# ohsnyt/bzip2-rust

Hardware: NVIDIA B200
Metric: compress_MBps_level9_byte_identical (higher is better)
Workload: dtype u8

## Files before the change

bzip2_rust_b200/csrc/bwt.cu:

```cuda
#include "common.cuh"
#include "sweep.cuh"

namespace {

constexpr int FB = 20;
constexpr u64 FMASK = (1ull << FB) - 1;
static_assert(BZ2B200_MAX_BLOCK < (1u << FB) - 1, "packed list fields are 20 bits");

constexpr int RT_IPT = 8;
constexpr int RT = BZ_THREADS * RT_IPT;
__device__ __forceinline__ u32 padi(u32 i) { return i + (i >> 5); }
constexpr int RT_PAD = RT + RT / 32 + 1;

#ifndef BZ_LW
#define BZ_LW 3072
#endif
constexpr int LW = BZ_LW;
constexpr int LIPT = LW / BZ_THREADS;
#ifndef BZ_LCAP
#define BZ_LCAP 1024
#endif
constexpr int LCAP = BZ_LCAP;
constexpr int LTILE = LW - LCAP;
#ifndef BZ_SCAP
// ... 60 lines not shown
            v.b = BSUM ? v.b + ob : max(v.b, ob);
            v.c += __shfl_xor_sync(0xffffffffu, v.c, o);
        }
        ex.a = max(ex.a, v.a); ex.b = BSUM ? ex.b + v.b : max(ex.b, v.b); ex.c += v.c;
        if (incm) break;
        hi -= 32;
    }
    Tri inc; inc.a = max(ex.a, agg.a); inc.b = BSUM ? ex.b + agg.b : max(ex.b, agg.b); inc.c = ex.c + agg.c;
    if (lane == 0) st_vol64(st + t, tri_pack(2, inc));
    return ex;
}

struct RefineArgs {
    const u8 *T; const u32 *len;
    const u32 *cnt;
    u32 *SA; u32 *RANK;
    const u64 *LIN; u64 *LOUT;
    u32 *cnt_out;
    u64 *LOUT2;
    u32 *cnt_out2;
    u64 *tstate;
    u32 *ticket;
    u32 stride, rtiles, tiles_x, nblk, group;
    u32 depth_after;
};

__device__ __forceinline__ bool ticket_tile(const RefineArgs &a, u32 *s_ticket, u32 &b, u32 &t) {
    if (threadIdx.x == 0) *s_ticket = atomicAdd(a.ticket, 1u);
    __syncthreads();
    u32 ticket = *s_ticket;
    u32 per_group = a.group * a.tiles_x;
    u32 g = ticket / per_group, r = ticket - g * per_group;
    t = r / a.group;
    b = g * a.group + (r - t * a.group);
    return b < a.nblk;
}

#ifndef BZ_REFINE_MINB
#define BZ_REFINE_MINB 5
#endif
__global__ void __launch_bounds__(BZ_THREADS, BZ_REFINE_MINB) k_init_ranks(RefineArgs a) {
    __shared__ u64 sk[RT + 2];
    __shared__ __align__(8) u8 fl[RT + 8];
    __shared__ u32 hd[RT_PAD];
    __shared__ u16 ls[RT];
    __shared__ int wsi[8];
    __shared__ u32 wsu[8];
    __shared__ u32 s_ticket;
    __shared__ Tri s_ex;
    __shared__ int s_big[2];
    u32 b, t;
    if (!ticket_tile(a, &s_ticket, b, t)) return;
    const u32 n = a.len[b];
    const u32 base = t * RT;
    if (base >= n) return;
    const int tid = threadIdx.x;
    const size_t ob = (size_t)b * a.stride;
    const u8 *Tb = a.T + ob;
    const u32 *sa = a.SA + ob;
    u32 s[RT_IPT];
#pragma unroll
    for (int r = 0; r < RT_IPT; r++) {
        u32 e = r * BZ_THREADS + tid, j = base + e;
        s[r] = 0;
        if (j < n) { s[r] = __ldg(sa + j); sk[e + 1] = rot_key8(Tb, n, s[r]); }
    }
    if (tid == 0 && base > 0) sk[0] = rot_key8(Tb, n, sa[base - 1]);
    if (tid == 32 && base + RT < n) sk[RT + 1] = rot_key8(Tb, n, sa[base + RT]);
    __syncthreads();
    for (u32 e = tid; e <= RT; e += BZ_THREADS) {
        u32 j = base + e;
        fl[e] = (j == 0 || j >= n || sk[e + 1] != sk[e]) ? 1 : 0;
    }
    __syncthreads();
    const u32 eb = tid * RT_IPT;
    const u64 f8 = *(const u64 *)(fl + eb);
    const u32 f9 = fl[eb + 8];
    u32 fm = 0;
#pragma unroll
    for (int r = 0; r < RT_IPT; r++) fm |= (u32)((f8 >> (8 * r)) & 1) << r;
    int last = -1;
    u32 hmask = 0, umask = 0;
#pragma unroll
    for (int r = 0; r < RT_IPT; r++) {
        u32 j = base + eb + r;
        bool h = (fm >> r) & 1;
        bool hn = (r == RT_IPT - 1) ? (f9 != 0) : ((fm >> (r + 1)) & 1);
        if (j < n) {
            if (h) { last = (int)j; hmask |= 1u << r; }
            if (!(h && hn)) umask |= 1u << r;
        }
    }
    int tl, fe;
    int head = block_excl_max(last, wsi, tl);
    int nxa = block_excl_min_rev(fm ? (int)(eb + __ffs(fm) - 1) : 0x7fffffff, wsi, fe);
    const bool cont = fl[RT] == 0;
    if (tid == 64) {
        int big = 0;
        if (fl[0] == 0) {
            if (fe == 0x7fffffff && cont) big = 1;
            else {
                long long E = (long long)base + (fe == 0x7fffffff ? (int)RT : fe);
                long long q = E - 1 - LCAP;
                if (q >= (long long)base) big = 1;
                else if (q >= 0) big = rot_key8(Tb, n, sa[q]) == sk[1];
            }
        }
        s_big[0] = big;
    }
    if (tid == 96) {
        int big = 0;
        if (cont) {
            if (tl < 0) big = 1;
            else {
                u32 P = (u32)tl + LCAP;
                if (P < base + RT) big = 1;
                else if (P < n) big = rot_key8(Tb, n, sa[P]) == sk[RT];
            }
        }
        s_big[1] = big;
    }
    __syncthreads();
    const int nx_out = f9 ? (int)(eb + 8) : (nxa != 0x7fffffff ? nxa : (cont ? 0x7fffffff : (int)RT));
    u32 bmask = 0, nloc = 0, nbig = 0;
#pragma unroll
    for (int r = 0; r < RT_IPT; r++) {
        if ((umask >> r) & 1) {
            u32 below = fm & ((2u << r) - 1u);
            int hh = below ? (int)(base + eb + 31 - __clz(below)) : head;
            u32 above = fm >> (r + 1);
            int nx = above ? (int)(eb + r + __ffs(above)) : nx_out;
            bool big;
            if (hh < 0) big = s_big[0] != 0;
            else if (nx == 0x7fffffff) big = s_big[1] != 0;
            else big = (int)base + nx - hh > LCAP;
            if (big) { bmask |= 1u << r; nbig++; } else nloc++;
        }
    }
    u32 tot;
    u32 kk = block_excl_sum(nloc | (nbig << 16), wsu, tot);
    const u32 tloc = tot & 0xffffu, tbig = tot >> 16;
    if (tid < 32) {
        Tri agg; agg.a = tl; agg.b = (int)tbig; agg.c = tloc;
        Tri ex = tile_lookback<true>(a.tstate + (size_t)b * a.rtiles, t, agg);
        if (tid == 0) {
            s_ex = ex;
            if (base + RT >= n) {
                bool done = a.depth_after >= n;
                a.cnt_out[b] = done ? 0u : ex.c + tloc;
                a.cnt_out2[b] = done ? 0u : (u32)ex.b + tbig;
            }
        }
    }
    __syncthreads();
    head = max(head, s_ex.a);
    u32 kl = kk & 0xffffu, kb = kk >> 16;
#pragma unroll
    for (int r = 0; r < RT_IPT; r++) {
        u32 e = eb + r;
        if ((hmask >> r) & 1) head = (int)(base + e);
        hd[padi(e)] = (u32)head;
        u16 v = 0xffff;
        if ((umask >> r) & 1) v = ((bmask >> r) & 1) ? (u16)(0x8000u | kb++) : (u16)(kl++);
        ls[e] = v;
    }
    __syncthreads();
    u32 *rank = a.RANK + ob;
    u64 *lout = a.LOUT + ob + s_ex.c;
    u64 *lout2 = a.LOUT2 + ob + (u32)s_ex.b;
#pragma unroll
    for (int r = 0; r < RT_IPT; r++) {
        u32 e = r * BZ_THREADS + tid, j = base + e;
        if (j < n) {
            u32 h = hd[padi(e)];
            rank[s[r]] = h;
            u32 slot = ls[e];
            if (slot != 0xffffu) {
                u64 v = ((u64)h << (2 * FB)) | s[r];
                if (slot & 0x8000u) lout2[slot & 0x7fffu] = v; else lout[slot] = v;
            }
        }
    }
}

template <bool HIST>
__global__ void __launch_bounds__(BZ_THREADS) k_list_key(const u32 *cntp, const u32 *len, const u32 *RANK, u64 *LIST,
                                                         u32 *counts, u32 stride, u32 h) {
    u32 b = blockIdx.y, cnt = cntp[b], n = len[b];
    u32 base = blockIdx.x * BZ_TILE;
    if (base >= cnt) return;
    __shared__ u32 hist[HIST ? 5 : 1][256];
    if (HIST) {
        for (int i = threadIdx.x; i < 5 * 256; i += BZ_THREADS) (&hist[0][0])[i] = 0;
        __syncthreads();
    }
    size_t ob = (size_t)b * stride;
    u64 *list = LIST + ob;
    const u32 *rank = RANK + ob;
    u32 hh = h >= n ? h % n : h;
#pragma unroll 4
    for (int r = 0; r < BZ_IPT; r++) {
        u32 k = base + r * BZ_THREADS + threadIdx.x;
        if (k < cnt) {
            u64 x = list[k];
            u32 p = (u32)(x & FMASK) + hh;
            if (p >= n) p -= n;
            x = (x & ~(FMASK << FB)) | ((u64)__ldg(rank + p) << FB);
            list[k] = x;
            if (HIST) {
#pragma unroll
                for (int q = 0; q < 5; q++) atomicAdd(&hist[q][(u32)(x >> (FB + 8 * q)) & 255u], 1u);
            }
        }
// ... 50 lines not shown
    u32 f9 = fl[eb + 8];
    int la = -1, lb = -1; u32 unres = 0;
    u32 smask = 0, gmask = 0, umask = 0;
#pragma unroll
    for (int r = 0; r < RT_IPT; r++) {
        u32 k = base + eb + r;
        u32 f = (u32)(f8 >> (8 * r)) & 3u;
        u32 fn = (r == RT_IPT - 1) ? f9 : ((u32)(f8 >> (8 * r + 8)) & 3u);
        if (k < cnt) {
            if (f & 2) { la = (int)k; gmask |= 1u << r; }
            if (f & 1) { lb = (int)k; smask |= 1u << r; }
            if (!((f & 1) && (fn & 1))) { unres++; umask |= 1u << r; }
        }
    }
    int ta, tb; u32 tu;
    int kg = block_excl_max(la, wsi, ta);
    int ks = block_excl_max(lb, wsi, tb);
    u32 ko = block_excl_sum(unres, wsu, tu);
    if (tid < 32) {
        Tri agg; agg.a = ta; agg.b = tb; agg.c = tu;
        Tri ex = tile_lookback(a.tstate + (size_t)b * a.rtiles, t, agg);
        if (tid == 0) {
            s_ex = ex;
            if (base + RT >= cnt) a.cnt_out[b] = (a.depth_after >= a.len[b]) ? 0u : ex.c + tu;
        }
    }
    __syncthreads();
    kg = max(kg, s_ex.a); ks = max(ks, s_ex.b);
    const u32 kbase = s_ex.c;
#pragma unroll
    for (int r = 0; r < RT_IPT; r++) {
        u32 e = eb + r;
        if ((gmask >> r) & 1) kg = (int)(base + e);
        if ((smask >> r) & 1) ks = (int)(base + e);
        kgs[padi(e)] = (u32)kg; kss[padi(e)] = (u32)ks;
        ls[e] = ((umask >> r) & 1) ? (u16)(ko++) : (u16)0xffff;
    }
    __syncthreads();
    u32 *sa = a.SA + ob, *rank = a.RANK + ob;
    u64 *lout = a.LOUT + ob + kbase;
#pragma unroll
    for (int r = 0; r < RT_IPT; r++) {
        u32 e = r * BZ_THREADS + tid, k = base + e;
        if (k < cnt) {
            u32 g = (u32)(x[r] >> (2 * FB));
            u32 s = (u32)(x[r] & FMASK);
            u32 kgv = kgs[padi(e)], ksv = kss[padi(e)];
            u32 nh = g + (ksv - kgv);
            sa[g + (k - kgv)] = s;
            rank[s] = nh;
            u32 slot = ls[e];
            if (slot != 0xffffu) lout[slot] = ((u64)nh << (2 * FB)) | s;
        }
    }
}

constexpr size_t LOC_K_BYTES = (size_t)LW * 4;
constexpr size_t LOC_I_BYTES = ((size_t)LWH * 2 + 15) & ~(size_t)15;
constexpr size_t LOC_G_BYTES = ((size_t)LWP * 4 + 15) & ~(size_t)15;
constexpr size_t LOC_U_BYTES = ((size_t)LWH * 2 + 15) & ~(size_t)15;
constexpr size_t LOC_W_BYTES = (size_t)(LW * 4 > 8 * 256 * 4 ? LW * 4 : 8 * 256 * 4);
constexpr size_t LOC_SMEM = LOC_K_BYTES + 2 * LOC_I_BYTES + LOC_G_BYTES + LOC_U_BYTES + LOC_W_BYTES;
static_assert(LOC_K_BYTES + 2 * LOC_I_BYTES >= (size_t)LW * 8, "staging area");
#ifndef BZ_LOCAL_MINB
#define BZ_LOCAL_MINB 3
#endif
__global__ void __launch_bounds__(BZ_THREADS, BZ_LOCAL_MINB) k_refine_local(RefineArgs a, u32 *err) {
    extern __shared__ __align__(16) u8 loc_smem[];
    u32 *K = (u32 *)loc_smem;
    u16 *IDXA = (u16 *)(loc_smem + LOC_K_BYTES);
    u16 *IDXB = (u16 *)(loc_smem + LOC_K_BYTES + LOC_I_BYTES);
    u32 *GSE = (u32 *)(loc_smem + LOC_K_BYTES + 2 * LOC_I_BYTES);
    u16 *UP = (u16 *)((u8 *)GSE + LOC_G_BYTES);
    u32 *wh = (u32 *)((u8 *)UP + LOC_U_BYTES);
    __shared__ u16 MG_GS[LW / (SCAP + 1) + 4], MG_MB[LW / (SCAP + 1) + 4];
    __shared__ int wsi[8];
    __shared__ u32 wsu[8];
    __shared__ u32 s_ticket, s_prevhead;
    __shared__ Tri s_ex;
    u32 b, t;
    if (!ticket_tile(a, &s_ticket, b, t)) return;
    const u32 cnt = a.cnt[b];
    const u32 base = t * LTILE;
    const int tid = threadIdx.x, lane = tid & 31, w = tid >> 5;
    if (cnt == 0 && t == 0 && tid == 0) a.cnt_out[b] = 0;
    if (base >= cnt) return;
    const size_t ob = (size_t)b * a.stride;
    const u64 *lin = a.LIN + ob + base;
// ... 167 lines not shown
            pk = k2;
            occ |= 1u << r;
        }
        occ &= (1u << LIPT) - 1u;
        const u32 own = sfm & ((1u << LIPT) - 1u);
        const u32 tm = occ & ~(own & (sfm >> 1));
        const int pin = block_excl_max(own ? (int)(eb + 31 - __clz(own)) : -1, wsi, dummy);
        u32 run = block_excl_sum((u32)__popc(tm), wsu, tu);
        int ps = pin;
#pragma unroll 4
        for (int r = 0; r < LIPT; r++) {
            u32 p = eb + r;
            if ((own >> r) & 1u) ps = (int)p;
            wh[p] = run | ((p - (u32)ps) << 12) | (((tm >> r) & 1u) << 31);
            run += (tm >> r) & 1u;
        }
    }
    __syncthreads();
    if (tid < 32) {
        Tri agg; agg.a = -1; agg.b = -1; agg.c = tu;
        Tri ex = tile_lookback(a.tstate + (size_t)b * a.rtiles, t, agg);
        if (tid == 0) {
            s_ex = ex;
            if (base + LTILE >= cnt) a.cnt_out[b] = (a.depth_after >= a.len[b]) ? 0u : ex.c + tu;
        }
    }
    u64 *stg = (u64 *)loc_smem;
    u32 *sa = a.SA + ob, *rank = a.RANK + ob;
#pragma unroll 2
    for (int r = 0; r < LIPT; r++) {
        u32 p = r * BZ_THREADS + tid;
        u32 e = UP[padh(p)];
        if (e != 0xffffu) {
            u32 gs = GSE[padi(e)] & 0xffffu;
            u32 v = wh[p];
            u64 x = __ldg(lin + e);
            u32 head = (u32)(x >> (2 * FB)), s = (u32)(x & FMASK);
            u32 off = p - gs;
            u32 nh = head + off - ((v >> 12) & 0x7ffffu);
            sa[head + off] = s;
            rank[s] = nh;
            if (v >> 31) stg[v & 0xfffu] = ((u64)nh << (2 * FB)) | s;
        }
    }
    __syncthreads();
    u64 *lout = a.LOUT + ob + s_ex.c;
    for (u32 q = tid; q < tu; q += BZ_THREADS) lout[q] = stg[q];
// ... 64 lines not shown
        if (e_ != cudaSuccess) { ctx->fail("kernel launch", e_, __FILE__, __LINE__); return BZ2B200_E_CUDA; } \
    } while (0)

int bz_bwt_batch(bz2b200_ctx *ctx, const Batch &B, u8 *d_bwt, u32 *d_key, u32 *d_usedbits) {
    if (B.nblk == 0) return BZ2B200_OK;
    if (B.max_n > BZ2B200_MAX_BLOCK || ((uintptr_t)B.T & 7u) || (B.stride & 7u)) { ctx->err = "bwt: bad batch geometry"; return BZ2B200_E_ARG; }
    cudaStream_t st = ctx->stream;
    const u64 ne_act = B.total_n;
    const size_t ne = (size_t)B.nblk * B.stride;
    const u32 min_tile = BZ_THREADS * 8;
    const u32 tiles_min = B.stride / min_tile;
    const u32 DSTRIDE = 8 * 256;
    const u32 NTICKET = 512;
    BZ_CHECK(ctx->d_SA.ensure(ne * 4));
    BZ_CHECK(ctx->d_SA2.ensure(ne * 4));
    BZ_CHECK(ctx->d_RANK.ensure(ne * 4));
    BZ_CHECK(ctx->d_KEYA.ensure(ne * 8));
    BZ_CHECK(ctx->d_KEYB.ensure(ne * 8));
    BZ_CHECK(ctx->d_thist.ensure((size_t)B.nblk * tiles_min * 256 * 4));
    BZ_CHECK(ctx->d_tagg.ensure((size_t)B.nblk * tiles_min * 8));
    BZ_CHECK(ctx->d_VALA.ensure(ne * 8));
    BZ_CHECK(ctx->d_VALB.ensure(ne * 8));
    BZ_CHECK(ctx->d_cnt.ensure((size_t)B.nblk * 4 * 4 + 16));
    BZ_CHECK(ctx->d_R.ensure(((size_t)B.nblk * DSTRIDE + NTICKET) * 4));
    BZ_CHECK(ctx->h_small.ensure((size_t)B.nblk * 8 + 64));
    u32 *d_sais = ctx->d_cnt.as<u32>() + (size_t)B.nblk * 4;
    BZ_CHECK(cudaMemsetAsync(d_sais, 0, 8, ctx->stream));
    if (!ctx->loc_attr_done) {
        BZ_CHECK(cudaFuncSetAttribute(k_refine_local, cudaFuncAttributeMaxDynamicSharedMemorySize, (int)LOC_SMEM));
        ctx->loc_attr_done = true;
    }
    u32 *SAa = ctx->d_SA.as<u32>(), *SAb = ctx->d_SA2.as<u32>(), *RANK = ctx->d_RANK.as<u32>();
    u64 *L0 = ctx->d_KEYA.as<u64>(), *L1 = ctx->d_KEYB.as<u64>();
    u64 *G0 = ctx->d_VALA.as<u64>(), *G1 = ctx->d_VALB.as<u64>();
    u32 *tstate = ctx->d_thist.as<u32>();
    u64 *rstate = ctx->d_tagg.as<u64>();
    u32 *dcounts = ctx->d_R.as<u32>();
    u32 *tickets = dcounts + (size_t)B.nblk * DSTRIDE;
    const size_t rstate_bytes = (size_t)B.nblk * tiles_min * 8;

    BZ_CHECK(cudaMemsetAsync(dcounts, 0, ((size_t)B.nblk * DSTRIDE + NTICKET) * 4, st));
    BZ_CHECK(cudaMemsetAsync(tstate, 0, (size_t)B.nblk * tiles_min * 256 * 4, st));
    u32 epoch = 0, tk = 0;
    dim3 gfull((B.max_n + BZ_TILE - 1) / BZ_TILE, B.nblk);
    static const u32 group_knob = [] { const char *e = getenv("BZ2B200_REFINE_GROUP"); u32 g = e ? (u32)atoi(e) : 4u; return g < 1 ? 1u : g; }();
    const u32 group = group_knob < (u32)B.nblk ? group_knob : (u32)B.nblk;

    ctx->prof_begin(K_BYTE_HIST, ne_act); sweep::k_byte_hist<<<gfull, BZ_THREADS, 0, st>>>(B.T, B.len, dcounts, B.stride, DSTRIDE); LAUNCH_OK();
    ctx->prof_begin(K_REF_PATH, (u64)B.nblk * 5000); k_ref_path<<<B.nblk, 128, 0, st>>>(B.T, B.len, B.stride, d_sais); LAUNCH_OK();
    if (d_usedbits) { ctx->prof_begin(K_USED, (u64)B.nblk * 1024); k_used_from_hist<<<B.nblk, 256, 0, st>>>(dcounts, DSTRIDE, d_usedbits); LAUNCH_OK(); }
    ctx->prof_begin(K_DIGIT_SCAN, (u64)B.nblk * DSTRIDE * 4); sweep::k_digit_scan<<<B.nblk * 8, 256, 0, st>>>(dcounts); LAUNCH_OK();
    u32 *bufs[2] = {SAa, SAb};
    const u32 *src = nullptr;
    for (int p = 0; p < 8; p++) {
        sweep::Args a{};
        a.T = B.T; a.len = B.len; a.cnt = B.len; a.in = src; a.out = bufs[p & 1];
        a.stride = B.stride; a.off = 7 - p; a.nblk = (u32)B.nblk;
        epoch++;
        a.dbase = dcounts; a.dbase_stride = DSTRIDE; a.tstate = tstate; a.ticket = tickets + tk++; a.epoch = epoch;
        if ((p & 1) == 0) { ctx->prof_begin(K_SWEEP_GATHER, ne_act * 9); sweep::launch<sweep::M_GATHER>(a, B.max_n, st); }
        else { ctx->prof_begin(K_SWEEP_CARRY, ne_act * 8); sweep::launch<sweep::M_CARRY>(a, B.max_n, st); }
        LAUNCH_OK();
        src = bufs[p & 1];
    }
    u32 *SA = bufs[1];

    u32 *cntL_cur = ctx->d_cnt.as<u32>(), *cntL_nxt = cntL_cur + B.nblk;
    u32 *cntB_cur = cntL_nxt + B.nblk, *cntB_nxt = cntB_cur + B.nblk;
    RefineArgs ra{};
    ra.T = B.T; ra.len = B.len; ra.SA = SA; ra.RANK = RANK; ra.stride = B.stride; ra.rtiles = tiles_min;
    ra.nblk = (u32)B.nblk; ra.group = group; ra.tstate = rstate;
    {
        BZ_CHECK(cudaMemsetAsync(rstate, 0, rstate_bytes, st));
        ra.cnt = B.len; ra.LIN = nullptr; ra.LOUT = L0; ra.cnt_out = cntL_cur; ra.LOUT2 = G0; ra.cnt_out2 = cntB_cur;
        ra.ticket = tickets + tk++;
        ra.tiles_x = (B.max_n + RT - 1) / RT; ra.depth_after = 8;
        u32 grid = ((ra.nblk + group - 1) / group) * group * ra.tiles_x;
        ctx->prof_begin(K_INIT_RANKS, ne_act * 16); k_init_ranks<<<grid, BZ_THREADS, 0, st>>>(ra); LAUNCH_OK();
    }

    u32 *h_cnt = ctx->h_small.as<u32>();
    const int passes = 5;
    u64 rounds = 0, listsum = 0, bigsum = 0;
    for (u32 h = 8;; h *= 2) {
        BZ_CHECK(cudaMemcpyAsync(h_cnt + 2 * B.nblk, d_sais, 8, cudaMemcpyDeviceToHost, st));
        BZ_CHECK(cudaMemcpyAsync(h_cnt, cntL_cur, (size_t)B.nblk * 4, cudaMemcpyDeviceToHost, st));
        BZ_CHECK(cudaMemcpyAsync(h_cnt + B.nblk, cntB_cur, (size_t)B.nblk * 4, cudaMemcpyDeviceToHost, st));
        BZ_CHECK(cudaStreamSynchronize(st));
        u32 maxl = 0, maxb = 0;
        u64 lsum = 0, bsum = 0;
        for (int b = 0; b < B.nblk; b++) {
            if (h_cnt[b] > maxl) maxl = h_cnt[b];
            if (h_cnt[B.nblk + b] > maxb) maxb = h_cnt[B.nblk + b];
            lsum += h_cnt[b]; bsum += h_cnt[B.nblk + b];
        }
        listsum += lsum + bsum; bigsum += bsum;
        if (maxl == 0 && maxb == 0) break;
        if (h >= (1u << 30)) { ctx->err = "bwt: doubling did not terminate"; return BZ2B200_E_CUDA; }
        rounds++;
        if (tk + (u32)passes + 3 > NTICKET) { BZ_CHECK(cudaMemsetAsync(tickets, 0, NTICKET * 4, st)); tk = 0; }
        if (maxl) {
            dim3 gl((maxl + BZ_TILE - 1) / BZ_TILE, B.nblk);
            ctx->prof_begin(K_LIST_KEY, lsum * 20); k_list_key<false><<<gl, BZ_THREADS, 0, st>>>(cntL_cur, B.len, RANK, L0, nullptr, B.stride, h); LAUNCH_OK();
            BZ_CHECK(cudaMemsetAsync(rstate, 0, rstate_bytes, st));
            ra.cnt = cntL_cur; ra.LIN = L0; ra.LOUT = L1; ra.cnt_out = cntL_nxt; ra.LOUT2 = nullptr; ra.cnt_out2 = nullptr;
            ra.ticket = tickets + tk++;
            ra.tiles_x = (maxl + LTILE - 1) / LTILE; ra.depth_after = 2 * h;
            u32 grid = ((ra.nblk + group - 1) / group) * group * ra.tiles_x;
            ctx->prof_begin(K_REFINE_LOCAL, lsum * 24); k_refine_local<<<grid, BZ_THREADS, LOC_SMEM, st>>>(ra, d_sais + 1); LAUNCH_OK();
            { u64 *tl = L0; L0 = L1; L1 = tl; }
        } else BZ_CHECK(cudaMemsetAsync(cntL_nxt, 0, (size_t)B.nblk * 4, st));
        if (maxb) {
            dim3 gl((maxb + BZ_TILE - 1) / BZ_TILE, B.nblk);
            BZ_CHECK(cudaMemsetAsync(dcounts, 0, (size_t)B.nblk * DSTRIDE * 4, st));
            ctx->prof_begin(K_LIST_KEY, bsum * 20); k_list_key<true><<<gl, BZ_THREADS, 0, st>>>(cntB_cur, B.len, RANK, G0, dcounts, B.stride, h); LAUNCH_OK();
            ctx->prof_begin(K_DIGIT_SCAN, (u64)B.nblk * DSTRIDE * 4); sweep::k_digit_scan<<<B.nblk * 8, 256, 0, st>>>(dcounts); LAUNCH_OK();
            if (epoch + (u32)passes > 254) {
                BZ_CHECK(cudaMemsetAsync(tstate, 0, (size_t)B.nblk * tiles_min * 256 * 4, st));
                epoch = 0;
            }
            for (int p = 0; p < passes; p++) {
                sweep::Args a{};
                a.T = B.T; a.len = B.len; a.cnt = cntB_cur; a.in = G0; a.out = G1;
                a.stride = B.stride; a.shift = FB + 8 * p; a.nblk = (u32)B.nblk;
                epoch++;
                a.dbase = dcounts + p * 256; a.dbase_stride = DSTRIDE; a.tstate = tstate; a.ticket = tickets + tk++; a.epoch = epoch;
                ctx->prof_begin(K_SWEEP_LIST, bsum * 16); sweep::launch<sweep::M_LIST>(a, maxb, st); LAUNCH_OK();
                u64 *tl = G0; G0 = G1; G1 = tl;
            }
            BZ_CHECK(cudaMemsetAsync(rstate, 0, rstate_bytes, st));
            ra.cnt = cntB_cur; ra.LIN = G0; ra.LOUT = G1; ra.cnt_out = cntB_nxt; ra.LOUT2 = nullptr; ra.cnt_out2 = nullptr;
            ra.ticket = tickets + tk++;
            ra.tiles_x = (maxb + RT - 1) / RT; ra.depth_after = 2 * h;
            u32 grid = ((ra.nblk + group - 1) / group) * group * ra.tiles_x;
            ctx->prof_begin(K_LIST_REFINE, bsum * 24); k_list_refine<<<grid, BZ_THREADS, 0, st>>>(ra); LAUNCH_OK();
            { u64 *tl = G0; G0 = G1; G1 = tl; }
        } else BZ_CHECK(cudaMemsetAsync(cntB_nxt, 0, (size_t)B.nblk * 4, st));
        { u32 *tc = cntL_cur; cntL_cur = cntL_nxt; cntL_nxt = tc; }
        { u32 *tc = cntB_cur; cntB_cur = cntB_nxt; cntB_nxt = tc; }
    }
    if (h_cnt[2 * B.nblk + 1]) { ctx->err = "bwt: a local group exceeded its capacity"; return BZ2B200_E_CUDA; }
    ctx->prof_begin(K_BWT_OUT, ne_act * 6); k_bwt_out<<<gfull, BZ_THREADS, 0, st>>>(B.T, B.len, SA, RANK, d_bwt, d_key, B.stride); LAUNCH_OK();
    ctx->bwt_stats[0] = (u64)B.nblk; ctx->bwt_stats[1] = ne_act; ctx->bwt_stats[2] = rounds; ctx->bwt_stats[3] = listsum;
    ctx->bwt_stats[4] = h_cnt[2 * B.nblk];
    ctx->bwt_stats[5] += h_cnt[2 * B.nblk];
    ctx->bwt_stats[6] += (u64)B.nblk;
    ctx->bwt_stats[7] = bigsum;
    return BZ2B200_OK;
}
```

bzip2_rust_b200/csrc/common.cuh:

```cuda
#pragma once
#include <cuda_runtime.h>
#include <stdint.h>
#include <stddef.h>
#include <mutex>
#include <string>
#include <vector>
#include <new>
#include "../../include/bz2b200.h"

typedef uint8_t u8;
typedef uint16_t u16;
typedef uint32_t u32;
typedef uint64_t u64;

#define BZ_CHECK(call)                                                                     \
    do {                                                                                   \
        cudaError_t e_ = (call);                                                           \
        if (e_ != cudaSuccess) {                                                           \
            ctx->fail(#call, e_, __FILE__, __LINE__);                                      \
            return BZ2B200_E_CUDA;                                                         \
        }                                                                                  \
    } while (0)

#define BZ_API_TRY try {
// ... 27 lines not shown
        return e;
    }
    void release() { if (p) cudaFreeHost(p); p = nullptr; cap = 0; }
    template <class T> T *as() const { return (T *)p; }
};

constexpr int BZ_THREADS = 256;
constexpr int BZ_IPT = 16;
constexpr int BZ_TILE = BZ_THREADS * BZ_IPT;
constexpr int BZ_GROUP = 50;
constexpr int BZ_MAXSYM = 258;

struct Batch {
    int nblk;
    u32 stride;
    u32 tiles;
    u32 max_n;
    int nbits;
    const u8 *T;
    const u32 *len;
    u64 total_n;
};

enum KernelId { K_RADIX_HIST0, K_RADIX_SCAN, K_RADIX_SCATTER0, K_REF_PATH, K_BYTE_HIST, K_DIGIT_SCAN, K_SWEEP_GATHER, K_SWEEP_CARRY, K_SWEEP_LIST, K_INIT_RANKS, K_LIST_KEY, K_LIST_REFINE, K_REFINE_LOCAL, K_BWT_OUT, K_USED, K_MTF_SUMMARY, K_MTF_SCAN, K_MTF_EMIT, K_HUF_INIT, K_HUF_SELECT, K_HUF_LENGTHS, K_HUF_GBITS, K_HUF_LAYOUT, K_HUF_EMIT, K_RLE_SCAN, K_RLE_CHAIN, K_RLE_EMIT, K_CRC_PIECES, K_CRC_FINAL, K_CONCAT, K_FOOTER, K_DEC_MISC, K_DEC_MAGIC, K_DEC_HEADER, K_DEC_JUMPS, K_DEC_BOUNDS, K_DEC_SYMS, K_DEC_CHUNKS, K_DEC_EXPAND, K_DEC_CHUNK_SCAN, K_IBWT_CHASE, K_IBWT_RANK, K_IBWT_WRITE, K_DEC_RLE1_COUNT, K_DEC_RLE1_WRITE, K_COUNT };
static const char *const kKernelNames[] = { "k_radix_hist0", "k_radix_scan", "k_radix_scatter0", "k_ref_path", "k_byte_hist", "k_digit_scan", "k_sweep_gather", "k_sweep_carry", "k_sweep_list", "k_init_ranks", "k_list_key", "k_list_refine", "k_refine_local", "k_bwt_out", "k_used", "k_mtf_summary", "k_mtf_scan", "k_mtf_emit", "k_huf_init", "k_huf_select", "k_huf_lengths", "k_huf_gbits", "k_huf_layout", "k_huf_emit", "k_rle_scan", "k_rle_chain", "k_rle_emit", "k_crc_pieces", "k_crc_final", "k_concat", "k_footer", "k_dec_misc", "k_dec_find_magic", "k_dec_header", "k_dec_jumps", "k_dec_bounds", "k_dec_syms", "k_dec_chunks", "k_dec_expand", "k_dec_chunk_scan", "k_ibwt_chase", "k_ibwt_rank", "k_ibwt_write", "k_dec_rle1_count", "k_dec_rle1_write" };

struct KStat { double ms = 0; u64 launches = 0; u64 bytes = 0; };
struct PendingEv { int id; u64 bytes; cudaEvent_t a, b; };

struct Arrival {
    std::vector<cudaEvent_t> *ev;
    size_t chunk;
    size_t win_off;
    size_t waited;
};

struct ShardPlan {
    bool scanned = false;
    const u8 *d_win = nullptr; size_t win_lo = 0, win_len = 0, n_total = 0; int level = 0;
    bool planned = false;
    bool eof = false; u32 off_from = 0, stop_rel = 0, s0 = 0, nb = 0;
};

struct bz2b200_ctx {
    int device = 0;
    ShardPlan shard;
    cudaStream_t stream = nullptr;
    cudaStream_t s_up = nullptr, s_down = nullptr;
// ... 157 lines not shown
```

bzip2_rust_b200/csrc/sweep.cuh:

```cuda
#pragma once
#include "common.cuh"
#include <stdlib.h>
#include <type_traits>

namespace sweep {

enum { M_GATHER = 0, M_LIST = 1, M_CARRY = 2 };

struct Args {
    const u8 *T; const u32 *len;
    const u32 *cnt;
    const void *in; void *out;
    const u32 *dbase;
    u32 dbase_stride;
    u32 *tstate;
    u32 *ticket;
    u32 stride;
    u32 rtiles;
    u32 epoch;
    u32 tiles_x;
    u32 nblk;
    u32 group;
    int off;
    int shift;
};

__device__ __forceinline__ u32 ld_vol(const u32 *p) {
    u32 v;
    asm volatile("ld.volatile.global.u32 %0, [%1];" : "=r"(v) : "l"(p));
    return v;
}
__device__ __forceinline__ void st_vol(u32 *p, u32 v) { asm volatile("st.volatile.global.u32 [%0], %1;" ::"l"(p), "r"(v) : "memory"); }

#ifndef BZ_SWEEP_TMA
#define BZ_SWEEP_TMA 0
#endif
__device__ __forceinline__ u32 smem_u32(const void *p) { return (u32)__cvta_generic_to_shared(p); }
__device__ __forceinline__ void mbar_init(u64 *bar, u32 count) {
    asm volatile("mbarrier.init.shared::cta.b64 [%0], %1;" ::"r"(smem_u32(bar)), "r"(count) : "memory");
    asm volatile("fence.mbarrier_init.release.cluster;" ::: "memory");
}
__device__ __forceinline__ void bulk_load(void *dst, const void *src, u32 bytes, u64 *bar) {
    asm volatile("mbarrier.arrive.expect_tx.shared::cta.b64 _, [%0], %1;" ::"r"(smem_u32(bar)), "r"(bytes) : "memory");
    asm volatile("cp.async.bulk.shared::cluster.global.mbarrier::complete_tx::bytes [%0], [%1], %2, [%3];"
// ... 152 lines not shown
__global__ void __launch_bounds__(BZ_THREADS, min_ctas(MODE, IPT)) k_sweep(Args a) {
    typedef typename Types<MODE>::Stage S;
    constexpr int TILE = BZ_THREADS * IPT;
    __shared__ u32 wh[8 * 256];
    __shared__ u32 toff[256];
    __shared__ u32 ws[8];
    __shared__ __align__(16) S sbuf[TILE];
    __shared__ __align__(8) u64 s_bar;
    __shared__ u32 s_ticket;
    const int tid = threadIdx.x;
    if (tid == 0) {
        s_ticket = atomicAdd(a.ticket, 1u);
        if (BZ_SWEEP_TMA && MODE != M_GATHER) mbar_init(&s_bar, 1);
    }
#pragma unroll
    for (int k = 0; k < 8; k++) wh[k * 256 + tid] = 0;
    __syncthreads();
    u32 ticket = s_ticket;
    u32 per_group = a.group * a.tiles_x;
    u32 g = ticket / per_group, r = ticket - g * per_group;
    u32 t = r / a.group;
    u32 b = g * a.group + (r - t * a.group);
    if (b >= a.nblk) return;
    u32 cnt = a.cnt[b];
    u32 base = t * TILE;
    if (base >= cnt) return;
    u32 n = a.len[b];
    u32 tile_n = min((u32)TILE, cnt - base);
    if (tile_n == (u32)TILE) {
        if (BZ_SWEEP_TMA && MODE != M_GATHER && tid == 0) {
            typedef typename Types<MODE>::In I;
            bulk_load(sbuf, (const I *)a.in + (size_t)b * a.stride + base, (u32)(TILE * sizeof(I)), &s_bar);
        }
        tile_body<MODE, IPT, true>(a, b, t, base, tile_n, n, wh, toff, ws, sbuf, &s_bar);
    } else tile_body<MODE, IPT, false>(a, b, t, base, tile_n, n, wh, toff, ws, sbuf, &s_bar);
}

struct Knobs { int ipt0, ipt1; u32 group, group_stream; };
static inline const Knobs &knobs() {
    static Knobs k = [] {
        Knobs q;
        const char *e;
        q.ipt0 = (e = getenv("BZ2B200_SWEEP_IPT0")) ? atoi(e) : 16;
        q.ipt1 = (e = getenv("BZ2B200_SWEEP_IPT1")) ? atoi(e) : 16;
        q.group = (e = getenv("BZ2B200_SWEEP_GROUP")) ? (u32)atoi(e) : 32u;
        q.group_stream = (e = getenv("BZ2B200_SWEEP_GROUP_STREAM")) ? (u32)atoi(e) : 128u;
// ... 56 lines not shown
```

Before: 7387.

## Pack alphabet-compressed multi-character keys for initial BWT suffix sort

For each block, maps the symbols that actually occur to dense codes and packs k consecutive characters into a base-sigma key of up to 44 bits. The initial suffix sort then runs as fewer 8-bit radix passes over these keys instead of eight byte passes, and prefix doubling starts at depth k instead of 8. Blocks are split into packed and legacy paths through block lists, and init_ranks reads keys from the packed rows. This adds a host synchronisation to read the pass count, extra planning kernels and per-block indirection. It also raises the occupancy hint on the local refine kernel.

Result: faster. 7886 (median of 6 runs) (+6.8%).

```diff
diff --git a/bzip2_rust_b200/csrc/bwt.cu b/bzip2_rust_b200/csrc/bwt.cu
--- a/bzip2_rust_b200/csrc/bwt.cu
+++ b/bzip2_rust_b200/csrc/bwt.cu
@@ -106,9 +106,13 @@
     u64 *tstate;
     u32 *ticket;
     u32 stride, rtiles, tiles_x, nblk, group;
-    u32 depth_after;
+    const u32 *blist;
+    const u32 *pinfo;
+    u32 dshift;
 };
-
+__device__ __forceinline__ u32 depth_after(const RefineArgs &a, u32 b) { return (a.pinfo[b] & 255u) << a.dshift; }
+
+template <bool BLIST = false>
 __device__ __forceinline__ bool ticket_tile(const RefineArgs &a, u32 *s_ticket, u32 &b, u32 &t) {
     if (threadIdx.x == 0) *s_ticket = atomicAdd(a.ticket, 1u);
     __syncthreads();
@@ -117,12 +121,118 @@
     u32 g = ticket / per_group, r = ticket - g * per_group;
     t = r / a.group;
     b = g * a.group + (r - t * a.group);
-    return b < a.nblk;
+    if (b >= a.nblk) return false;
+    if (BLIST && a.blist) b = a.blist[b];
+    return true;
+}
+
+#ifndef BZ_PK_BITS
+#define BZ_PK_BITS 44
+#endif
+constexpr int PK_BITS = BZ_PK_BITS;
+constexpr u32 PK_MAXK = 32;
+constexpr int PK_PASSES = (PK_BITS + 7) / 8;
+static_assert(PK_BITS <= 64 - FB && 1 + PK_PASSES <= 8, "packed key geometry");
+
+__global__ void __launch_bounds__(256) k_pack_plan(u32 *counts, u32 cstride, const u32 *len, int mode, u8 *codes,
+                                                   u32 *pinfo, u32 *cntP, u32 *cntG, u32 *summary) {
+    __shared__ u32 ws[8];
+    const u32 b = blockIdx.x, c = threadIdx.x;
+    u32 *row = counts + (size_t)b * cstride;
+    u32 sigma;
+    const u32 code = block_excl_sum(row[c] != 0 ? 1u : 0u, ws, sigma);
+    codes[(size_t)b * 256 + c] = (u8)code;
+    const u32 n = len[b];
+    u32 k = PK_MAXK;
+    u64 pw = 1;
+    if (sigma > 1) {
+        k = 0;
+        while (k < PK_MAXK && pw * sigma <= (1ull << PK_BITS)) { pw *= sigma; k++; }
+    }
+    const u32 passes = pw > 1 ? (u32)(64 - __clzll((long long)(pw - 1)) + 7) / 8 : 0u;
+    const bool packed = mode != 0 && k >= 8 && n > 0;
+    if (c == 0) {
+        pinfo[b] = packed ? (k | passes << 8 | sigma << 16) : (8u | sigma << 16);
+        cntP[b] = packed ? n : 0u;
+        cntG[b] = packed ? 0u : n;
+        if (packed) atomicMax(summary, passes);
+    }
+    if (packed && c >= passes && c < (u32)PK_PASSES) row[(1 + c) * 256] = n;
+}
+
+__global__ void __launch_bounds__(256) k_path_lists(const u32 *cntP, const u32 *cntG, u32 nblk, u32 *listP, u32 *listG,
+                                                    u32 *summary) {
+    __shared__ u32 ws[8], ws2[8];
+    u32 np = 0, ng = 0;
+    for (u32 c0 = 0; c0 < nblk; c0 += 256) {
+        const u32 b = c0 + threadIdx.x;
+        const u32 p = b < nblk && cntP[b] != 0, g = b < nblk && cntG[b] != 0;
+        u32 tp, tg;
+        const u32 xp = block_excl_sum(p, ws, tp), xg = block_excl_sum(g, ws2, tg);
+        if (p) listP[np + xp] = b;
+        if (g) listG[ng + xg] = b;
+        np += tp; ng += tg;
+    }
+    if (threadIdx.x == 0) { summary[1] = ng; summary[2] = np; }
+}
+
+constexpr int PK_RUN = 16;
+static_assert(BZ_TILE == BZ_THREADS * PK_RUN, "one run per thread");
+__global__ void __launch_bounds__(BZ_THREADS) k_pack_keys(const u8 *T, const u32 *listP, const u32 *cntP, const u8 *codes,
+                                                          const u32 *pinfo, u64 *out, u32 *counts, u32 stride, u32 cstride) {
+    const u32 b = listP ? listP[blockIdx.y] : blockIdx.y, n = cntP[b];
+    const u32 base = blockIdx.x * BZ_TILE;
+    if (base >= n) return;
+    __shared__ u8 cd[256];
+    __shared__ u8 tc[BZ_TILE + PK_MAXK];
+    __shared__ u32 hist[PK_PASSES][256];
+    __shared__ u64 stage[BZ_TILE + BZ_TILE / PK_RUN];
+    const int tid = threadIdx.x;
+    const u32 info = pinfo[b], k = info & 255u, np = (info >> 8) & 255u, sigma = info >> 16;
+    cd[tid] = codes[(size_t)b * 256 + tid];
+    for (int i = tid; i < PK_PASSES * 256; i += BZ_THREADS) (&hist[0][0])[i] = 0;
+    __syncthreads();
+    const u8 *Tb = T + (size_t)b * stride;
+    const u32 tile_n = min((u32)BZ_TILE, n - base);
+    for (u32 i = tid; i < tile_n + k - 1; i += BZ_THREADS) {
+        u32 p = base + i;
+        if (p >= n) p %= n;
+        tc[i] = cd[__ldg(Tb + p)];
+    }
+    u64 top = 1;
+    for (u32 q = 1; q < k; q++) top *= sigma;
+    __syncthreads();
+    const u32 e0 = tid * PK_RUN;
+    u64 key = 0;
+    if (e0 < tile_n)
+        for (u32 q = 0; q < k; q++) key = key * sigma + tc[e0 + q];
+#pragma unroll
+    for (int i = 0; i < PK_RUN; i++) {
+        const u32 e = e0 + i;
+        if (e < tile_n) {
+            if (i) key = (key - top * tc[e - 1]) * sigma + tc[e + k - 1];
+            const u64 x = (key << FB) | (base + e);
+            stage[e + e / PK_RUN] = x;
+            for (u32 p = 0; p < np; p++) atomicAdd(&hist[p][(u32)(x >> (FB + 8 * p)) & 255u], 1u);
+        }
+    }
+    __syncthreads();
+    u64 *o = out + (size_t)b * stride + base;
+#pragma unroll 4
+    for (int r = 0; r < PK_RUN; r++) {
+        const u32 e = r * BZ_THREADS + tid;
+        if (e < tile_n) o[e] = stage[e + e / PK_RUN];
+    }
+    for (u32 i = tid; i < np * 256; i += BZ_THREADS) {
+        const u32 v = (&hist[0][0])[i];
+        if (v) atomicAdd(&counts[(size_t)b * cstride + 256 + i], v);
+    }
 }
 
 #ifndef BZ_REFINE_MINB
 #define BZ_REFINE_MINB 5
 #endif
+template <bool PACKED>
 __global__ void __launch_bounds__(BZ_THREADS, BZ_REFINE_MINB) k_init_ranks(RefineArgs a) {
     __shared__ u64 sk[RT + 2];
     __shared__ __align__(8) u8 fl[RT + 8];
@@ -134,23 +244,32 @@
     __shared__ Tri s_ex;
     __shared__ int s_big[2];
     u32 b, t;
-    if (!ticket_tile(a, &s_ticket, b, t)) return;
-    const u32 n = a.len[b];
+    if (!ticket_tile<true>(a, &s_ticket, b, t)) return;
+    const u32 n = a.cnt[b];
     const u32 base = t * RT;
     if (base >= n) return;
     const int tid = threadIdx.x;
     const size_t ob = (size_t)b * a.stride;
     const u8 *Tb = a.T + ob;
     const u32 *sa = a.SA + ob;
+    const u64 *rows = a.LIN + ob;
+    auto row_key = [&](u32 j) -> u64 { return PACKED ? __ldg(rows + j) >> FB : rot_key8(Tb, n, __ldg(sa + j)); };
     u32 s[RT_IPT];
 #pragma unroll
     for (int r = 0; r < RT_IPT; r++) {
         u32 e = r * BZ_THREADS + tid, j = base + e;
         s[r] = 0;
-        if (j < n) { s[r] = __ldg(sa + j); sk[e + 1] = rot_key8(Tb, n, s[r]); }
-    }
-    if (tid == 0 && base > 0) sk[0] = rot_key8(Tb, n, sa[base - 1]);
-    if (tid == 32 && base + RT < n) sk[RT + 1] = rot_key8(Tb, n, sa[base + RT]);
+        if (j < n) {
+            if (PACKED) {
+                u64 x = __ldg(rows + j);
+                s[r] = (u32)(x & FMASK);
+                sk[e + 1] = x >> FB;
+                a.SA[ob + j] = s[r];
+            } else { s[r] = __ldg(sa + j); sk[e + 1] = rot_key8(Tb, n, s[r]); }
+        }
+    }
+    if (tid == 0 && base > 0) sk[0] = row_key(base - 1);
+    if (tid == 32 && base + RT < n) sk[RT + 1] = row_key(base + RT);
     __syncthreads();
     for (u32 e = tid; e <= RT; e += BZ_THREADS) {
         u32 j = base + e;
@@ -187,7 +306,7 @@
                 long long E = (long long)base + (fe == 0x7fffffff ? (int)RT : fe);
                 long long q = E - 1 - LCAP;
                 if (q >= (long long)base) big = 1;
-                else if (q >= 0) big = rot_key8(Tb, n, sa[q]) == sk[1];
+                else if (q >= 0) big = row_key((u32)q) == sk[1];
             }
         }
         s_big[0] = big;
@@ -199,7 +318,7 @@
             else {
                 u32 P = (u32)tl + LCAP;
                 if (P < base + RT) big = 1;
-                else if (P < n) big = rot_key8(Tb, n, sa[P]) == sk[RT];
+                else if (P < n) big = row_key(P) == sk[RT];
             }
         }
         s_big[1] = big;
@@ -230,7 +349,7 @@
         if (tid == 0) {
             s_ex = ex;
             if (base + RT >= n) {
-                bool done = a.depth_after >= n;
+                bool done = depth_after(a, b) >= n;
                 a.cnt_out[b] = done ? 0u : ex.c + tloc;
                 a.cnt_out2[b] = done ? 0u : (u32)ex.b + tbig;
             }
@@ -269,10 +388,11 @@
 
 template <bool HIST>
 __global__ void __launch_bounds__(BZ_THREADS) k_list_key(const u32 *cntp, const u32 *len, const u32 *RANK, u64 *LIST,
-                                                         u32 *counts, u32 stride, u32 h) {
+                                                         u32 *counts, u32 stride, const u32 *pinfo, u32 round) {
     u32 b = blockIdx.y, cnt = cntp[b], n = len[b];
     u32 base = blockIdx.x * BZ_TILE;
     if (base >= cnt) return;
+    const u32 h = (pinfo[b] & 255u) << round;
     __shared__ u32 hist[HIST ? 5 : 1][256];
     if (HIST) {
         for (int i = threadIdx.x; i < 5 * 256; i += BZ_THREADS) (&hist[0][0])[i] = 0;
@@ -369,7 +489,7 @@
         Tri ex = tile_lookback(a.tstate + (size_t)b * a.rtiles, t, agg);
         if (tid == 0) {
             s_ex = ex;
-            if (base + RT >= cnt) a.cnt_out[b] = (a.depth_after >= a.len[b]) ? 0u : ex.c + tu;
+            if (base + RT >= cnt) a.cnt_out[b] = (depth_after(a, b) >= a.len[b]) ? 0u : ex.c + tu;
         }
     }
     __syncthreads();
@@ -410,7 +530,7 @@
 constexpr size_t LOC_SMEM = LOC_K_BYTES + 2 * LOC_I_BYTES + LOC_G_BYTES + LOC_U_BYTES + LOC_W_BYTES;
 static_assert(LOC_K_BYTES + 2 * LOC_I_BYTES >= (size_t)LW * 8, "staging area");
 #ifndef BZ_LOCAL_MINB
-#define BZ_LOCAL_MINB 3
+#define BZ_LOCAL_MINB 4
 #endif
 __global__ void __launch_bounds__(BZ_THREADS, BZ_LOCAL_MINB) k_refine_local(RefineArgs a, u32 *err) {
     extern __shared__ __align__(16) u8 loc_smem[];
@@ -624,7 +744,7 @@
         Tri ex = tile_lookback(a.tstate + (size_t)b * a.rtiles, t, agg);
         if (tid == 0) {
             s_ex = ex;
-            if (base + LTILE >= cnt) a.cnt_out[b] = (a.depth_after >= a.len[b]) ? 0u : ex.c + tu;
+            if (base + LTILE >= cnt) a.cnt_out[b] = (depth_after(a, b) >= a.len[b]) ? 0u : ex.c + tu;
         }
     }
     u64 *stg = (u64 *)loc_smem;
@@ -735,7 +855,8 @@
     BZ_CHECK(ctx->d_VALA.ensure(ne * 8));
     BZ_CHECK(ctx->d_VALB.ensure(ne * 8));
     BZ_CHECK(ctx->d_cnt.ensure((size_t)B.nblk * 4 * 4 + 16));
-    BZ_CHECK(ctx->d_R.ensure(((size_t)B.nblk * DSTRIDE + NTICKET) * 4));
+    const u32 NSUM = 4;
+    BZ_CHECK(ctx->d_R.ensure(((size_t)B.nblk * DSTRIDE + NTICKET + NSUM + (size_t)B.nblk * (5 + 64)) * 4));
     BZ_CHECK(ctx->h_small.ensure((size_t)B.nblk * 8 + 64));
     u32 *d_sais = ctx->d_cnt.as<u32>() + (size_t)B.nblk * 4;
     BZ_CHECK(cudaMemsetAsync(d_sais, 0, 8, ctx->stream));
@@ -750,9 +871,13 @@
     u64 *rstate = ctx->d_tagg.as<u64>();
     u32 *dcounts = ctx->d_R.as<u32>();
     u32 *tickets = dcounts + (size_t)B.nblk * DSTRIDE;
+    u32 *d_summary = tickets + NTICKET;
+    u32 *pinfo = d_summary + NSUM, *cntP = pinfo + B.nblk, *cntG = cntP + B.nblk;
+    u32 *listP = cntG + B.nblk, *listG = listP + B.nblk;
+    u8 *codes = (u8 *)(listG + B.nblk);
     const size_t rstate_bytes = (size_t)B.nblk * tiles_min * 8;
 
-    BZ_CHECK(cudaMemsetAsync(dcounts, 0, ((size_t)B.nblk * DSTRIDE + NTICKET) * 4, st));
+    BZ_CHECK(cudaMemsetAsync(dcounts, 0, ((size_t)B.nblk * DSTRIDE + NTICKET + NSUM) * 4, st));
     BZ_CHECK(cudaMemsetAsync(tstate, 0, (size_t)B.nblk * tiles_min * 256 * 4, st));
     u32 epoch = 0, tk = 0;
     dim3 gfull((B.max_n + BZ_TILE - 1) / BZ_TILE, B.nblk);
@@ -760,15 +885,31 @@
     const u32 group = group_knob < (u32)B.nblk ? group_knob : (u32)B.nblk;
 
     ctx->prof_begin(K_BYTE_HIST, ne_act); sweep::k_byte_hist<<<gfull, BZ_THREADS, 0, st>>>(B.T, B.len, dcounts, B.stride, DSTRIDE); LAUNCH_OK();
+    static const int pack_mode = [] { const char *e = getenv("BZ2B200_BWT_PACKED"); return e ? atoi(e) : 1; }();
+    ctx->prof_begin(K_PACK_PLAN, (u64)B.nblk * 1024);
+    k_pack_plan<<<B.nblk, 256, 0, st>>>(dcounts, DSTRIDE, B.len, pack_mode, codes, pinfo, cntP, cntG, d_summary); LAUNCH_OK();
+    ctx->prof_begin(K_PACK_PLAN, (u64)B.nblk * 16);
+    k_path_lists<<<1, 256, 0, st>>>(cntP, cntG, (u32)B.nblk, listP, listG, d_summary); LAUNCH_OK();
+    u32 *h_cnt = ctx->h_small.as<u32>();
+    u32 *h_sum = h_cnt + 2 * B.nblk + 4;
+    BZ_CHECK(cudaMemcpyAsync(h_sum, d_summary, NSUM * 4, cudaMemcpyDeviceToHost, st));
     ctx->prof_begin(K_REF_PATH, (u64)B.nblk * 5000); k_ref_path<<<B.nblk, 128, 0, st>>>(B.T, B.len, B.stride, d_sais); LAUNCH_OK();
     if (d_usedbits) { ctx->prof_begin(K_USED, (u64)B.nblk * 1024); k_used_from_hist<<<B.nblk, 256, 0, st>>>(dcounts, DSTRIDE, d_usedbits); LAUNCH_OK(); }
+    BZ_CHECK(cudaStreamSynchronize(st));
+    const u32 key_passes = h_sum[0], n_legacy = h_sum[1], n_packed = h_sum[2];
+    const u32 *lG = n_legacy == (u32)B.nblk ? nullptr : listG, *lP = n_packed == (u32)B.nblk ? nullptr : listP;
+    if (n_packed) {
+        ctx->prof_begin(K_PACK_KEYS, ne_act * 9);
+        k_pack_keys<<<dim3(gfull.x, n_packed), BZ_THREADS, 0, st>>>(B.T, lP, cntP, codes, pinfo, L1, dcounts, B.stride, DSTRIDE);
+        LAUNCH_OK();
+    }
     ctx->prof_begin(K_DIGIT_SCAN, (u64)B.nblk * DSTRIDE * 4); sweep::k_digit_scan<<<B.nblk * 8, 256, 0, st>>>(dcounts); LAUNCH_OK();
     u32 *bufs[2] = {SAa, SAb};
     const u32 *src = nullptr;
-    for (int p = 0; p < 8; p++) {
+    for (int p = 0; p < (n_legacy ? 8 : 0); p++) {
         sweep::Args a{};
-        a.T = B.T; a.len = B.len; a.cnt = B.len; a.in = src; a.out = bufs[p & 1];
-        a.stride = B.stride; a.off = 7 - p; a.nblk = (u32)B.nblk;
+        a.T = B.T; a.len = B.len; a.cnt = cntG; a.in = src; a.out = bufs[p & 1];
+        a.stride = B.stride; a.off = 7 - p; a.nblk = n_legacy; a.blist = lG;
         epoch++;
         a.dbase = dcounts; a.dbase_stride = DSTRIDE; a.tstate = tstate; a.ticket = tickets + tk++; a.epoch = epoch;
         if ((p & 1) == 0) { ctx->prof_begin(K_SWEEP_GATHER, ne_act * 9); sweep::launch<sweep::M_GATHER>(a, B.max_n, st); }
@@ -777,25 +918,46 @@
         src = bufs[p & 1];
     }
     u32 *SA = bufs[1];
+    u64 *pk = L1, *pk_alt = G1;
+    for (u32 p = 0; p < key_passes; p++) {
+        sweep::Args a{};
+        a.T = B.T; a.len = B.len; a.cnt = cntP; a.in = pk; a.out = pk_alt;
+        a.stride = B.stride; a.shift = FB + 8 * (int)p; a.nblk = n_packed; a.blist = lP;
+        epoch++;
+        a.dbase = dcounts + (1 + p) * 256; a.dbase_stride = DSTRIDE; a.tstate = tstate; a.ticket = tickets + tk++; a.epoch = epoch;
+        ctx->prof_begin(K_SWEEP_KEY, ne_act * 16); sweep::launch<sweep::M_LIST>(a, B.max_n, st); LAUNCH_OK();
+        u64 *tp = pk; pk = pk_alt; pk_alt = tp;
+    }
 
     u32 *cntL_cur = ctx->d_cnt.as<u32>(), *cntL_nxt = cntL_cur + B.nblk;
     u32 *cntB_cur = cntL_nxt + B.nblk, *cntB_nxt = cntB_cur + B.nblk;
     RefineArgs ra{};
     ra.T = B.T; ra.len = B.len; ra.SA = SA; ra.RANK = RANK; ra.stride = B.stride; ra.rtiles = tiles_min;
-    ra.nblk = (u32)B.nblk; ra.group = group; ra.tstate = rstate;
+    ra.nblk = (u32)B.nblk; ra.group = group; ra.tstate = rstate; ra.pinfo = pinfo;
     {
         BZ_CHECK(cudaMemsetAsync(rstate, 0, rstate_bytes, st));
-        ra.cnt = B.len; ra.LIN = nullptr; ra.LOUT = L0; ra.cnt_out = cntL_cur; ra.LOUT2 = G0; ra.cnt_out2 = cntB_cur;
-        ra.ticket = tickets + tk++;
-        ra.tiles_x = (B.max_n + RT - 1) / RT; ra.depth_after = 8;
-        u32 grid = ((ra.nblk + group - 1) / group) * group * ra.tiles_x;
-        ctx->prof_begin(K_INIT_RANKS, ne_act * 16); k_init_ranks<<<grid, BZ_THREADS, 0, st>>>(ra); LAUNCH_OK();
-    }
-
-    u32 *h_cnt = ctx->h_small.as<u32>();
+        ra.LOUT = L0; ra.cnt_out = cntL_cur; ra.LOUT2 = G0; ra.cnt_out2 = cntB_cur;
+        ra.tiles_x = (B.max_n + RT - 1) / RT; ra.dshift = 0;
+        auto path_grid = [&](u32 nb, const u32 *list) {
+            ra.nblk = nb; ra.blist = list; ra.group = group_knob < nb ? group_knob : nb;
+            return ((nb + ra.group - 1) / ra.group) * ra.group * ra.tiles_x;
+        };
+        if (n_legacy) {
+            u32 grid = path_grid(n_legacy, lG);
+            ra.cnt = cntG; ra.LIN = nullptr; ra.ticket = tickets + tk++;
+            ctx->prof_begin(K_INIT_RANKS, ne_act * 16); k_init_ranks<false><<<grid, BZ_THREADS, 0, st>>>(ra); LAUNCH_OK();
+        }
+        if (n_packed) {
+            u32 grid = path_grid(n_packed, lP);
+            ra.cnt = cntP; ra.LIN = pk; ra.ticket = tickets + tk++;
+            ctx->prof_begin(K_INIT_RANKS, ne_act * 16); k_init_ranks<true><<<grid, BZ_THREADS, 0, st>>>(ra); LAUNCH_OK();
+        }
+        ra.nblk = (u32)B.nblk; ra.blist = nullptr; ra.group = group;
+    }
+
     const int passes = 5;
     u64 rounds = 0, listsum = 0, bigsum = 0;
-    for (u32 h = 8;; h *= 2) {
+    for (u32 r = 0;; r++) {
         BZ_CHECK(cudaMemcpyAsync(h_cnt + 2 * B.nblk, d_sais, 8, cudaMemcpyDeviceToHost, st));
         BZ_CHECK(cudaMemcpyAsync(h_cnt, cntL_cur, (size_t)B.nblk * 4, cudaMemcpyDeviceToHost, st));
         BZ_CHECK(cudaMemcpyAsync(h_cnt + B.nblk, cntB_cur, (size_t)B.nblk * 4, cudaMemcpyDeviceToHost, st));
@@ -809,16 +971,16 @@
         }
         listsum += lsum + bsum; bigsum += bsum;
         if (maxl == 0 && maxb == 0) break;
-        if (h >= (1u << 30)) { ctx->err = "bwt: doubling did not terminate"; return BZ2B200_E_CUDA; }
+        if (r >= 26) { ctx->err = "bwt: doubling did not terminate"; return BZ2B200_E_CUDA; }
         rounds++;
         if (tk + (u32)passes + 3 > NTICKET) { BZ_CHECK(cudaMemsetAsync(tickets, 0, NTICKET * 4, st)); tk = 0; }
         if (maxl) {
             dim3 gl((maxl + BZ_TILE - 1) / BZ_TILE, B.nblk);
-            ctx->prof_begin(K_LIST_KEY, lsum * 20); k_list_key<false><<<gl, BZ_THREADS, 0, st>>>(cntL_cur, B.len, RANK, L0, nullptr, B.stride, h); LAUNCH_OK();
+            ctx->prof_begin(K_LIST_KEY, lsum * 20); k_list_key<false><<<gl, BZ_THREADS, 0, st>>>(cntL_cur, B.len, RANK, L0, nullptr, B.stride, pinfo, r); LAUNCH_OK();
             BZ_CHECK(cudaMemsetAsync(rstate, 0, rstate_bytes, st));
             ra.cnt = cntL_cur; ra.LIN = L0; ra.LOUT = L1; ra.cnt_out = cntL_nxt; ra.LOUT2 = nullptr; ra.cnt_out2 = nullptr;
             ra.ticket = tickets + tk++;
-            ra.tiles_x = (maxl + LTILE - 1) / LTILE; ra.depth_after = 2 * h;
+            ra.tiles_x = (maxl + LTILE - 1) / LTILE; ra.dshift = r + 1;
             u32 grid = ((ra.nblk + group - 1) / group) * group * ra.tiles_x;
             ctx->prof_begin(K_REFINE_LOCAL, lsum * 24); k_refine_local<<<grid, BZ_THREADS, LOC_SMEM, st>>>(ra, d_sais + 1); LAUNCH_OK();
             { u64 *tl = L0; L0 = L1; L1 = tl; }
@@ -826,7 +988,7 @@
         if (maxb) {
             dim3 gl((maxb + BZ_TILE - 1) / BZ_TILE, B.nblk);
             BZ_CHECK(cudaMemsetAsync(dcounts, 0, (size_t)B.nblk * DSTRIDE * 4, st));
-            ctx->prof_begin(K_LIST_KEY, bsum * 20); k_list_key<true><<<gl, BZ_THREADS, 0, st>>>(cntB_cur, B.len, RANK, G0, dcounts, B.stride, h); LAUNCH_OK();
+            ctx->prof_begin(K_LIST_KEY, bsum * 20); k_list_key<true><<<gl, BZ_THREADS, 0, st>>>(cntB_cur, B.len, RANK, G0, dcounts, B.stride, pinfo, r); LAUNCH_OK();
             ctx->prof_begin(K_DIGIT_SCAN, (u64)B.nblk * DSTRIDE * 4); sweep::k_digit_scan<<<B.nblk * 8, 256, 0, st>>>(dcounts); LAUNCH_OK();
             if (epoch + (u32)passes > 254) {
                 BZ_CHECK(cudaMemsetAsync(tstate, 0, (size_t)B.nblk * tiles_min * 256 * 4, st));
@@ -844,7 +1006,7 @@
             BZ_CHECK(cudaMemsetAsync(rstate, 0, rstate_bytes, st));
             ra.cnt = cntB_cur; ra.LIN = G0; ra.LOUT = G1; ra.cnt_out = cntB_nxt; ra.LOUT2 = nullptr; ra.cnt_out2 = nullptr;
             ra.ticket = tickets + tk++;
-            ra.tiles_x = (maxb + RT - 1) / RT; ra.depth_after = 2 * h;
+            ra.tiles_x = (maxb + RT - 1) / RT; ra.dshift = r + 1;
             u32 grid = ((ra.nblk + group - 1) / group) * group * ra.tiles_x;
             ctx->prof_begin(K_LIST_REFINE, bsum * 24); k_list_refine<<<grid, BZ_THREADS, 0, st>>>(ra); LAUNCH_OK();
             { u64 *tl = G0; G0 = G1; G1 = tl; }
diff --git a/bzip2_rust_b200/csrc/common.cuh b/bzip2_rust_b200/csrc/common.cuh
--- a/bzip2_rust_b200/csrc/common.cuh
+++ b/bzip2_rust_b200/csrc/common.cuh
@@ -73,8 +73,9 @@
     u64 total_n;
 };
 
-enum KernelId { K_RADIX_HIST0, K_RADIX_SCAN, K_RADIX_SCATTER0, K_REF_PATH, K_BYTE_HIST, K_DIGIT_SCAN, K_SWEEP_GATHER, K_SWEEP_CARRY, K_SWEEP_LIST, K_INIT_RANKS, K_LIST_KEY, K_LIST_REFINE, K_REFINE_LOCAL, K_BWT_OUT, K_USED, K_MTF_SUMMARY, K_MTF_SCAN, K_MTF_EMIT, K_HUF_INIT, K_HUF_SELECT, K_HUF_LENGTHS, K_HUF_GBITS, K_HUF_LAYOUT, K_HUF_EMIT, K_RLE_SCAN, K_RLE_CHAIN, K_RLE_EMIT, K_CRC_PIECES, K_CRC_FINAL, K_CONCAT, K_FOOTER, K_DEC_MISC, K_DEC_MAGIC, K_DEC_HEADER, K_DEC_JUMPS, K_DEC_BOUNDS, K_DEC_SYMS, K_DEC_CHUNKS, K_DEC_EXPAND, K_DEC_CHUNK_SCAN, K_IBWT_CHASE, K_IBWT_RANK, K_IBWT_WRITE, K_DEC_RLE1_COUNT, K_DEC_RLE1_WRITE, K_COUNT };
-static const char *const kKernelNames[] = { "k_radix_hist0", "k_radix_scan", "k_radix_scatter0", "k_ref_path", "k_byte_hist", "k_digit_scan", "k_sweep_gather", "k_sweep_carry", "k_sweep_list", "k_init_ranks", "k_list_key", "k_list_refine", "k_refine_local", "k_bwt_out", "k_used", "k_mtf_summary", "k_mtf_scan", "k_mtf_emit", "k_huf_init", "k_huf_select", "k_huf_lengths", "k_huf_gbits", "k_huf_layout", "k_huf_emit", "k_rle_scan", "k_rle_chain", "k_rle_emit", "k_crc_pieces", "k_crc_final", "k_concat", "k_footer", "k_dec_misc", "k_dec_find_magic", "k_dec_header", "k_dec_jumps", "k_dec_bounds", "k_dec_syms", "k_dec_chunks", "k_dec_expand", "k_dec_chunk_scan", "k_ibwt_chase", "k_ibwt_rank", "k_ibwt_write", "k_dec_rle1_count", "k_dec_rle1_write" };
+enum KernelId { K_RADIX_HIST0, K_RADIX_SCAN, K_RADIX_SCATTER0, K_REF_PATH, K_BYTE_HIST, K_DIGIT_SCAN, K_SWEEP_GATHER, K_SWEEP_CARRY, K_SWEEP_LIST, K_INIT_RANKS, K_LIST_KEY, K_LIST_REFINE, K_REFINE_LOCAL, K_BWT_OUT, K_PACK_PLAN, K_PACK_KEYS, K_SWEEP_KEY, K_USED, K_MTF_SUMMARY, K_MTF_SCAN, K_MTF_EMIT, K_HUF_INIT, K_HUF_SELECT, K_HUF_LENGTHS, K_HUF_GBITS, K_HUF_LAYOUT, K_HUF_EMIT, K_RLE_SCAN, K_RLE_CHAIN, K_RLE_EMIT, K_CRC_PIECES, K_CRC_FINAL, K_CONCAT, K_FOOTER, K_DEC_MISC, K_DEC_MAGIC, K_DEC_HEADER, K_DEC_JUMPS, K_DEC_BOUNDS, K_DEC_SYMS, K_DEC_CHUNKS, K_DEC_EXPAND, K_DEC_CHUNK_SCAN, K_IBWT_CHASE, K_IBWT_RANK, K_IBWT_WRITE, K_DEC_RLE1_COUNT, K_DEC_RLE1_WRITE, K_COUNT };
+static const char *const kKernelNames[] = { "k_radix_hist0", "k_radix_scan", "k_radix_scatter0", "k_ref_path", "k_byte_hist", "k_digit_scan", "k_sweep_gather", "k_sweep_carry", "k_sweep_list", "k_init_ranks", "k_list_key", "k_list_refine", "k_refine_local", "k_bwt_out", "k_pack_plan", "k_pack_keys", "k_sweep_key", "k_used", "k_mtf_summary", "k_mtf_scan", "k_mtf_emit", "k_huf_init", "k_huf_select", "k_huf_lengths", "k_huf_gbits", "k_huf_layout", "k_huf_emit", "k_rle_scan", "k_rle_chain", "k_rle_emit", "k_crc_pieces", "k_crc_final", "k_concat", "k_footer", "k_dec_misc", "k_dec_find_magic", "k_dec_header", "k_dec_jumps", "k_dec_bounds", "k_dec_syms", "k_dec_chunks", "k_dec_expand", "k_dec_chunk_scan", "k_ibwt_chase", "k_ibwt_rank", "k_ibwt_write", "k_dec_rle1_count", "k_dec_rle1_write" };
+static_assert(sizeof(kKernelNames) / sizeof(kKernelNames[0]) == K_COUNT, "one name per kernel id");
 
 struct KStat { double ms = 0; u64 launches = 0; u64 bytes = 0; };
 struct PendingEv { int id; u64 bytes; cudaEvent_t a, b; };
diff --git a/bzip2_rust_b200/csrc/sweep.cuh b/bzip2_rust_b200/csrc/sweep.cuh
--- a/bzip2_rust_b200/csrc/sweep.cuh
+++ b/bzip2_rust_b200/csrc/sweep.cuh
@@ -20,6 +20,7 @@
     u32 epoch;
     u32 tiles_x;
     u32 nblk;
+    const u32 *blist;
     u32 group;
     int off;
     int shift;
@@ -218,6 +219,7 @@
     u32 t = r / a.group;
     u32 b = g * a.group + (r - t * a.group);
     if (b >= a.nblk) return;
+    if (a.blist) b = a.blist[b];
     u32 cnt = a.cnt[b];
     u32 base = t * TILE;
     if (base >= cnt) return;
```
